# ErlerPhilipp/points2surf

Measured on AMD Instinct MI355X. Metric: SDF queries/sec/GPU (p2s_max, 256^3 grid), higher is better.
Workload: dtype f32

## Files before the change

### include/p2s_hip.h

```cpp
#ifndef P2S_HIP_H
#define P2S_HIP_H

#include <stddef.h>
#include <stdint.h>

#ifdef __cplusplus
extern "C" {
#endif

#define P2S_ABI_VERSION 5

#define P2S_OK            0
#define P2S_EINVAL       -1
#define P2S_EHIP         -2
#define P2S_ENOMEM       -3
#define P2S_ECAPACITY    -4
#define P2S_ENODEVICE    -5
#define P2S_EIO          -6

typedef struct p2s_model_s *p2s_model_t;
typedef struct p2s_cloud_s *p2s_cloud_t;
typedef struct p2s_rng_s   *p2s_rng_t;
typedef struct p2s_trimesh_s *p2s_trimesh_t;

// ... 125 lines not shown
    const p2s_rng_t *sub;
    const p2s_rng_t *first;
} p2s_worker_streams;
int p2s_stream_order(int64_t first_position, int64_t n, int n_streams, int batch, const float *q_in_dev, float *q_out_dev,
                     int64_t *src_out_dev, int64_t *counts_host, void *stream);
int p2s_infer_shape_workers(p2s_model_t m, p2s_cloud_t c, const p2s_worker_streams *ws, int grid_resolution, int epsilon,
                            int64_t q_begin, int64_t q_end, int chunk, float *sdf_out_dev, float *q_out_dev, int64_t *n_done,
                            void *stream);
int p2s_infer_queries_workers(p2s_model_t m, p2s_cloud_t c, const p2s_worker_streams *ws, int rotate, const float *q_dev,
                              int64_t n_queries, int chunk, float *sdf_out_dev, void *stream);
int p2s_subsample_workers(p2s_cloud_t c, const p2s_worker_streams *ws, const float *q_dev, int64_t n_queries, int n, int weighted,
                          int32_t *ids_out_dev, float *pts_out_dev, void *stream);
int p2s_model_capture_logits(p2s_model_t m, float *logits_out_dev, int64_t capacity_queries);
int p2s_debug_fault_chunk(p2s_model_t m, int chunk_index);
int p2s_debug_stn_pool(p2s_model_t m, int n_queries, float *out_dev, void *stream);

int p2s_sdf_volume(const float *query_dev, const float *sdf_dev, int64_t n, int grid_res, int sigma,
                   float certainty_threshold, int clamp, int device, float *vol_out_dev, int32_t *iterations,
                   void *stream);

int p2s_marching_cubes(const float *vol_dev, int grid_res, float *verts_out_dev, int64_t cap_verts,
                       int32_t *faces_out_dev, int64_t cap_faces, int64_t *n_verts, int64_t *n_faces,
                       int model_space, int fix_inversion, int *inverted, int device, void *stream);
int p2s_mc_cell(const float *values8, int32_t *row, int32_t *n_tri, int32_t *edges36);

int p2s_rng_random_sample(p2s_rng_t r, int64_t n, double *out_dev, void *stream);
int p2s_mesh_sample_surface(const float *verts_dev, const int32_t *faces_dev, int64_t n_faces, const double *u_dev,
                            int64_t n_samples, float *pts_out_dev, int32_t *face_out_dev, double *area_host,
                            int device, void *stream);
int p2s_points_remove_close(const float *pts_dev, int64_t m, double radius, int64_t limit, float *pts_out_dev,
// ... 61 lines not shown
                       int64_t *info_host, void *stream);

int p2s_write_txt_f32(const char *path, const float *values_host, int64_t n);
int p2s_write_query_vis_ply(const char *path, const float *query_host, const float *dist_host, int64_t n);
int p2s_write_coff_samples(const char *path, const float *query_host, const float *dist_host, int64_t n);

typedef struct {
    double  ms_chain_stn, ms_stn_head, ms_chain_main, ms_decoder, ms_knn, ms_subsample, ms_grid;
    int64_t queries;
    int64_t launches_chain;
    double  ms_chain_qstn;
    int64_t fallback_queries;
    int64_t conv3_confirmed;
    int64_t conv3_items_dense;
    int64_t conv3_items;
    double  reserved[3];
} p2s_counters;
int p2s_set_profiling(p2s_model_t m, int enabled);
int p2s_get_counters(p2s_model_t m, p2s_counters *out);

typedef struct p2s_trainer_s *p2s_trainer_t;

int p2s_trainer_create(const p2s_model_cfg *cfg, int use_feat_stn, const float *params_host, int64_t n_params,
                       const float *buffers_host, int64_t n_buffers, int64_t num_batches_tracked, int device,
                       p2s_trainer_t *out);
int p2s_trainer_destroy(p2s_trainer_t t);
int p2s_trainer_sizes(p2s_trainer_t t, int64_t *n_params, int64_t *n_buffers, int64_t *n_pools, int64_t *resident_bytes);
int p2s_trainer_forward_backward(p2s_trainer_t t, const float *patch_ps_dev, const float *sub_ms_dev, const float *query_dev,
                                 const float *dist_abs_dev, const float *sign01_dev, const float *radius_dev, int B,
                                 double *losses_host, void *stream);
int p2s_trainer_sgd_step(p2s_trainer_t t, double lr, double momentum, void *stream);
// ... 21 lines not shown
```

### points2surf_amd/_lib.py

```python
import ctypes
import os

from .weights import ModelCfg, WeightOffsets

HERE = os.path.dirname(os.path.abspath(__file__))
LIB_PATH = os.environ.get('P2S_LIB_PATH') or os.path.join(HERE, 'libp2s_hip.so')

P2S_OK = 0
P2S_ECAPACITY = -4

c_void_p = ctypes.c_void_p
c_int = ctypes.c_int
c_int64 = ctypes.c_int64


class Counters(ctypes.Structure):
    _fields_ = [('ms_chain_stn', ctypes.c_double), ('ms_stn_head', ctypes.c_double),
                ('ms_chain_main', ctypes.c_double), ('ms_decoder', ctypes.c_double),
                ('ms_knn', ctypes.c_double), ('ms_subsample', ctypes.c_double), ('ms_grid', ctypes.c_double),
                ('queries', ctypes.c_int64), ('launches_chain', ctypes.c_int64),
                ('ms_chain_qstn', ctypes.c_double), ('fallback_queries', ctypes.c_int64),
                ('conv3_confirmed', ctypes.c_int64), ('conv3_items_dense', ctypes.c_int64), ('conv3_items', ctypes.c_int64),
                ('reserved', ctypes.c_double * 3)]


PROTOTYPES = {
    'p2s_abi_version': (c_int, []),
    'p2s_last_error': (ctypes.c_char_p, []),
    'p2s_device_count': (c_int, []),
    'p2s_release_scratch': (c_int, [c_int]),
    'p2s_model_create': (c_int, [ctypes.POINTER(ModelCfg), c_void_p, ctypes.c_size_t,
                                 ctypes.POINTER(WeightOffsets), c_int, ctypes.POINTER(c_void_p)]),
    'p2s_model_destroy': (c_int, [c_void_p]),
    'p2s_encode_decode': (c_int, [c_void_p, c_void_p, c_void_p, c_void_p, c_void_p, c_int, c_void_p, c_void_p,
                                  c_void_p]),
    'p2s_encode_features': (c_int, [c_void_p, c_void_p, c_void_p, c_void_p, c_int, c_void_p, c_void_p, c_void_p]),
    'p2s_cloud_create': (c_int, [c_void_p, c_int, c_int, c_void_p, ctypes.POINTER(c_void_p)]),
    'p2s_cloud_destroy': (c_int, [c_void_p]),
# ... 16 lines not shown
    'p2s_patch_from_ids': (c_int, [c_void_p, c_void_p, c_void_p, c_void_p, c_int64, c_int, c_void_p, c_void_p, c_void_p]),
    'p2s_gather_points': (c_int, [c_void_p, c_void_p, c_int64, c_void_p, c_void_p]),
    'p2s_infer_shape': (c_int, [c_void_p, c_void_p, c_void_p, c_int, c_int, c_int64, c_int64, c_int, c_void_p,
                                c_void_p, ctypes.POINTER(c_int64), c_void_p]),
    'p2s_infer_shape_ball': (c_int, [c_void_p, c_void_p, c_void_p, c_void_p, c_int, c_int, c_int64, c_int64, c_int, c_void_p,
                                     c_void_p, ctypes.POINTER(c_int64), c_void_p]),
    'p2s_kd_order_host': (c_int, [c_void_p, c_int64, c_int, c_void_p, c_void_p, c_int64, ctypes.POINTER(ctypes.c_int32)]),
    'p2s_ball_count': (c_int, [c_void_p, c_void_p, c_int64, ctypes.c_double, c_void_p, c_void_p]),
    'p2s_ball_patch': (c_int, [c_void_p, c_void_p, c_void_p, c_int64, ctypes.c_double, c_int, c_int, c_void_p, c_void_p,
                               c_void_p, c_void_p, c_void_p]),
    'p2s_infer_queries': (c_int, [c_void_p, c_void_p, c_void_p, c_void_p, c_void_p, c_int64, c_int, c_void_p, c_void_p]),
    'p2s_random_rotations': (c_int, [c_void_p, c_int64, c_void_p, c_void_p]),
    'p2s_rotate_points': (c_int, [c_void_p, c_void_p, c_int, c_int64, c_void_p, c_void_p]),
    'p2s_debug_fault_chunk': (c_int, [c_void_p, c_int]),
    'p2s_debug_stn_pool': (c_int, [c_void_p, c_int, c_void_p, c_void_p]),
    'p2s_sdf_volume': (c_int, [c_void_p, c_void_p, c_int64, c_int, c_int, ctypes.c_float, c_int, c_int, c_void_p,
                               ctypes.POINTER(ctypes.c_int32), c_void_p]),
    'p2s_marching_cubes': (c_int, [c_void_p, c_int, c_void_p, c_int64, c_void_p, c_int64, ctypes.POINTER(c_int64),
                                   ctypes.POINTER(c_int64), c_int, c_int, ctypes.POINTER(c_int), c_int, c_void_p]),
    'p2s_mc_cell': (c_int, [c_void_p, ctypes.POINTER(ctypes.c_int32), ctypes.POINTER(ctypes.c_int32), c_void_p]),
    'p2s_rng_random_sample': (c_int, [c_void_p, c_int64, c_void_p, c_void_p]),
    'p2s_mesh_sample_surface': (c_int, [c_void_p, c_void_p, c_int64, c_void_p, c_int64, c_void_p, c_void_p,
                                        ctypes.POINTER(ctypes.c_double), c_int, c_void_p]),
    'p2s_points_remove_close': (c_int, [c_void_p, c_int64, ctypes.c_double, c_int64, c_void_p, ctypes.POINTER(c_int64), c_int,
                                        c_void_p]),
    'p2s_nn_distance_stats': (c_int, [c_void_p, c_void_p, c_int64, c_void_p, ctypes.POINTER(ctypes.c_double),
                                      ctypes.POINTER(ctypes.c_double), c_void_p]),
    'p2s_trimesh_create': (c_int, [c_void_p, c_int64, c_void_p, c_int64, c_int, c_void_p, ctypes.POINTER(c_void_p)]),
    'p2s_trimesh_destroy': (c_int, [c_void_p]),
    'p2s_trimesh_info': (c_int, [c_void_p, ctypes.POINTER(c_int64)]),
# ... 97 lines not shown
```

### points2surf_amd/build.py

```python
import glob
import os
import subprocess
import sys

HERE = os.path.dirname(os.path.abspath(__file__))
CSRC = os.path.join(HERE, 'csrc')
LIB = os.path.join(HERE, 'libp2s_hip.so')


def hipcc_path():
    for c in (os.environ.get('HIPCC'), '/opt/rocm/bin/hipcc', 'hipcc'):
        if c and (os.path.isfile(c) or c == 'hipcc'):
            return c
    return 'hipcc'


def sources():
    return sorted(glob.glob(os.path.join(CSRC, '*.hip')))


def needs_build():
    if not os.path.isfile(LIB):
        return True
    t = os.path.getmtime(LIB)
# ... 21 lines not shown
    tag = hashlib.sha1(' '.join(flags).encode()).hexdigest()[:10]
    todo, objs = [], []
    for src in sources():
        obj = os.path.join(objdir, '%s.%s.o' % (os.path.basename(src)[:-4], tag))
        objs.append(obj)
        if force or not os.path.isfile(obj) or os.path.getmtime(obj) < max(os.path.getmtime(src), hdr_time):
            todo.append((src, obj))

    def compile_one(job):
        src, obj = job
        cmd = [hipcc_path()] + flags + ['-c', src, '-o', obj]
        if verbose:
            print(' '.join(cmd), flush=True)
        subprocess.check_call(cmd)

    jobs = jobs or int(os.environ.get('P2S_BUILD_JOBS', min(8, os.cpu_count() or 1)))
    with concurrent.futures.ThreadPoolExecutor(max_workers=max(1, jobs)) as ex:
        list(ex.map(compile_one, todo))
    cmd = [hipcc_path(), '--offload-arch=gfx950', '-shared', '-fPIC', '-fno-gpu-rdc', '-o', LIB] + objs
    if verbose:
        print(' '.join(cmd), flush=True)
    subprocess.check_call(cmd)
    return LIB


if __name__ == '__main__':
    build(force='--force' in sys.argv)
    print(LIB)
```

### points2surf_amd/csrc/p2s_api.hip

```cpp
#include "p2s_common.h"
#include "p2s_internal.h"
#include <vector>
#include <cstring>
#include <algorithm>
#include <mutex>
#include <cstdlib>

static thread_local char g_err[512] = "";

void p2s_set_error(const char *fmt, ...) {
    va_list ap;
    va_start(ap, fmt);
    vsnprintf(g_err, sizeof(g_err), fmt, ap);
    va_end(ap);
}

namespace {
struct DevScratch {
    std::mutex mu;
    void *p = nullptr;
    size_t cap = 0;
};
DevScratch g_scratch[P2S_MAX_DEVICES];
}
// ... 58 lines not shown
    const p2s_model_cfg &cfg = m->cfg;
    hipError_t e = hipMalloc(&m->blob, n_floats * sizeof(float));
    if (e != hipSuccess) {
        p2s_set_error("hipMalloc(weights) failed: %s", hipGetErrorString(e));
        return P2S_ENOMEM;
    }
    e = hipMemcpy(m->blob, blob_host, n_floats * sizeof(float), hipMemcpyHostToDevice);
    if (e != hipSuccess) {
        p2s_set_error("hipMemcpy(weights) failed: %s", hipGetErrorString(e));
        return P2S_EHIP;
    }
    const Precision prec = p2s_precision(cfg);
    {
        const int rc = screen_init(m);
        if (rc) return rc;
    }
    if (!prec.pieces) return P2S_OK;
    struct Item { P2sLayer layer; int z; };
    std::vector<Item> items;
    for (int kind = LK_ENC; kind < LK_FP32; ++kind) {
        if (!p2s_kind_packed((P2sLayerKind)kind, cfg)) continue;
        const int slices = kind == LK_ENC || kind == LK_ENC_HEAD ? 2 : 1;
        for (int z = 0; z < slices; ++z)
            for (int l = 0; l < P2S_LAYERS; ++l) {
                if (p2s_layers[l].kind != kind) continue;
                m->h_off[l][z] = m->h_off[l][1] = m->h_total;
                items.push_back({(P2sLayer)l, z});
                m->h_total += (size_t)p2s_layers[l].K * p2s_layers[l].N;
            }
    }
// ... 123 lines not shown
    if (m->aux) (void)hipStreamDestroy(m->aux);
    if (m->ball) (void)hipStreamDestroy(m->ball);
    delete m;
    return P2S_OK;
}

int p2s_set_profiling(p2s_model_t m, int enabled) {
    if (!m) return P2S_EINVAL;
    m->profiling = enabled != 0;
    return P2S_OK;
}

int p2s_get_counters(p2s_model_t m, p2s_counters *out) {
    if (!m || !out) return P2S_EINVAL;
    *out = m->counters;
    if (m->scr_counters) {
        unsigned long long h[3] = {};
        P2S_HIP_CHECK(hipSetDevice(m->device));
        P2S_HIP_CHECK(hipMemcpy(h, m->scr_counters, sizeof(h), hipMemcpyDeviceToHost));
        out->conv3_confirmed = (int64_t)h[0];
        out->conv3_items_dense = (int64_t)h[1];
        out->conv3_items = (int64_t)h[2];
    }
    return P2S_OK;
}

}

int p2s_prof_mark(p2s_model_s *m, hipStream_t s) {
    if (!m->profiling) return -1;
// ... 132 lines not shown
```

### points2surf_amd/csrc/p2s_chain.hip

```cpp
#include "p2s_common.h"
#include <cstdlib>
#include <atomic>

namespace {

constexpr int MT = 64;
constexpr int SA = 68;
constexpr int SB = 132;

__device__ __forceinline__ f32x16 mfma32(float a, float b, f32x16 c) {
    return __builtin_amdgcn_mfma_f32_32x32x2f32(a, b, c, 0, 0, 0);
}

__device__ __forceinline__ f32x4 ldg4(const float *p) { return *reinterpret_cast<const f32x4 *>(p); }
__device__ __forceinline__ f32x4 lds4(const float *p) { return *reinterpret_cast<const f32x4 *>(p); }
__device__ __forceinline__ f32x4 bufld4(__amdgpu_buffer_rsrc_t rsrc, int voff, int soff) {
    typedef unsigned u32x4 __attribute__((ext_vector_type(4)));
    const u32x4 v = __builtin_amdgcn_raw_buffer_load_b128(rsrc, voff, soff, 0);
    f32x4 r;
    r[0] = __uint_as_float(v[0]); r[1] = __uint_as_float(v[1]); r[2] = __uint_as_float(v[2]); r[3] = __uint_as_float(v[3]);
    return r;
}

__device__ __forceinline__ void store_tile_bias_relu(const f32x16 &acc, float *dst, int stride, int row0,
                                                     int col0, const float *__restrict__ bias, int lane) {
    const int col = col0 + (lane & 31);
    const float b = bias[col];
    const int rbase = row0 + 4 * (lane >> 5);
#pragma unroll
    for (int reg = 0; reg < 16; ++reg) {
        const int row = rbase + (reg & 3) + 8 * (reg >> 2);
        dst[row * stride + col] = fmaxf(acc[reg] + b, 0.0f);
    }
}

__device__ __forceinline__ f32x16 zero16() {
    f32x16 z;
#pragma unroll
    for (int i = 0; i < 16; ++i) z[i] = 0.0f;
    return z;
}

struct B8 {
    f32x4 v[8];
};
__device__ __forceinline__ void load_b8(B8 &b, __amdgpu_buffer_rsrc_t rsrc, int lane16, int soff) {
#pragma unroll
    for (int kg = 0; kg < 8; ++kg) b.v[kg] = bufld4(rsrc, lane16, soff + kg * 1024);
// ... 103 lines not shown
    const auto r = __builtin_amdgcn_permlane32_swap(u, u, false, false);
    return __uint_as_float(r[0]) + __uint_as_float(r[1]);
}

typedef unsigned int u32x4 __attribute__((ext_vector_type(4)));
typedef _Float16 f16x8 __attribute__((ext_vector_type(8)));
typedef _Float16 f16x2 __attribute__((ext_vector_type(2)));
typedef float f32x2 __attribute__((ext_vector_type(2)));
constexpr int SCR_HB = 128 + 8;
constexpr int SCR_QCAP = 256;
constexpr float P2S_SCR_KAPPA = 0x1.1p-10f;
constexpr int SCR_OFF_E = MT * SA + MT * SB;
constexpr int SCR_OFF_Q = SCR_OFF_E + 1024;
constexpr int SCR_OFF_RED = SCR_OFF_Q + 4 * SCR_QCAP;
constexpr int SCR_LDS_FLOATS = SCR_OFF_RED + 8;
static_assert(MT * SCR_HB * 2 <= MT * SA * 4, "the fp16 copy fits the 64-channel tile it lies over");
static_assert(2 * SCR_LDS_FLOATS * 4 <= 160 * 1024, "two workgroups per CU");

__device__ __forceinline__ u32x4 scr_bufld(__amdgpu_buffer_rsrc_t rsrc, int voff, int soff) {
    return __builtin_amdgcn_raw_buffer_load_b128(rsrc, voff, soff, 0);
}
__device__ __forceinline__ u32x4 scr_lds_a(const unsigned short *buf, int row0, int kb, int lane) {
    return *reinterpret_cast<const u32x4 *>(buf + (row0 + (lane & 31)) * SCR_HB + 16 * kb + 8 * (lane >> 5));
}
__device__ __forceinline__ f32x16 scr_mfma(u32x4 a, u32x4 b, f32x16 c) {
    return __builtin_amdgcn_mfma_f32_32x32x16_f16(__builtin_bit_cast(f16x8, a), __builtin_bit_cast(f16x8, b), c, 0, 0, 0);
}
__device__ __forceinline__ unsigned scr_half2(float a, float b) {
    const f32x2 v = {a, b};
    return __builtin_bit_cast(unsigned, __builtin_convertvector(v, f16x2));
}
constexpr int SCR_CDEPTH = 4;
// ... 51 lines not shown
    const int wave = __builtin_amdgcn_readfirstlane(tid >> 6);

    int item = blockIdx.x;
    int bsel = 0;
    if (item >= args.br[0].n_items) {
        item -= args.br[0].n_items;
        bsel = 1;
    }
    const ChainBranch &br = args.br[bsel];
    const int P = br.P, P1 = br.P1;
    const float *__restrict__ w0a = br.w0a;
    const float *__restrict__ b0a = br.b0a;
    const float *__restrict__ w1 = br.w1 + (long long)item * br.w1_item_stride;
    const float *__restrict__ w3 = br.w3;
    const bool short_chain = br.short_chain != 0;

    float cx = 0.f, cy = 0.f, cz = 0.f;
    if (br.center) {
        cx = br.center[item * 3 + 0];
        cy = br.center[item * 3 + 1];
        cz = br.center[item * 3 + 2];
    }
    float R[9];
    const bool has_rot = br.rot != nullptr;
    if (has_rot) {
#pragma unroll
        for (int i = 0; i < 9; ++i) R[i] = br.rot[item * 9 + i];
    }

    const float pool0 = SUM ? 0.0f : -INFINITY;
// ... 31 lines not shown
    float *scr_red = smem + SCR_OFF_RED;
    unsigned *scr_q = reinterpret_cast<unsigned *>(smem + SCR_OFF_Q) + SCR_QCAP * wave;
    const float *__restrict__ scr_mu = args.w3mu[bsel];
    const __amdgpu_buffer_rsrc_t rs3h = __builtin_amdgcn_make_buffer_rsrc(const_cast<unsigned short *>(args.w3h[bsel]), 0,
                                                                           (int)(P2S_SCR_PIECE * 2), 0x00020000);
    float sr0 = -INFINITY, sr1 = -INFINITY, sr2 = -INFINITY, sr3 = -INFINITY, sr4 = -INFINITY, sr5 = -INFINITY, sr6 = -INFINITY,
          sr7 = -INFINITY;
    bool undec = false;
    float scr_Hsq = 0.0f;
    int nconf = 0;
    bool dense_pass = !SCREEN;
    if constexpr (SCREEN) {
#pragma unroll
        for (int i = 0; i < 4; ++i) scr_E[64 * i + lane] = __float_as_uint(-INFINITY);
    }
    for (;;) {
    load_point(0, nx0, nx1, nx2);
    for (int tile = 0; tile < ntiles; ++tile) {
      if constexpr (SCREEN) {
          asm volatile("" : "+v"(tid));
          lane = tid & 63;
          lane16 = lane * 16;
      }
      f32x4 bA0, bA1, aA0, aA1, bB0, bB1, aB0, aB1;
      if (ablate != 1) {
        float x0 = nx0, x1 = nx1, x2 = nx2;
        B8 wb;
        if (!short_chain) load_b8(wb, rs0b, lane16, (wave & 1) * 8192);
        else load_b8(wb, rs2, lane16, wave * 8192);
        if (has_rot) {
#pragma clang fp contract(off)
            const float y0 = __builtin_fmaf(R[0], x0, R[1] * x1) + R[2] * x2;
            const float y1 = __builtin_fmaf(R[5], x2, __builtin_fmaf(R[3], x0, R[4] * x1));
            const float y2 = __builtin_fmaf(R[8], x2, __builtin_fmaf(R[6], x0, R[7] * x1));
            x0 = y0; x1 = y1; x2 = y2;
        }
        bad = bad || !(fabsf(x0) <= 3.0e38f) || !(fabsf(x1) <= 3.0e38f) || !(fabsf(x2) <= 3.0e38f);
        {
            float *dst = bufA + lane * SA + 16 * wave;
#pragma unroll
            for (int c4 = 0; c4 < 4; ++c4) {
                f32x4 v;
#pragma unroll
                for (int c = 0; c < 4; ++c) {
                    const int o = 16 * wave + 4 * c4 + c;
                    float s = b0a[o];
                    s = fmaf(w0a[o], x0, s);
                    s = fmaf(w0a[64 + o], x1, s);
                    s = fmaf(w0a[128 + o], x2, s);
                    v[c] = fmaxf(s, 0.0f);
                }
                *reinterpret_cast<f32x4 *>(dst + 4 * c4) = v;
            }
        }
        __syncthreads();

        if (!short_chain) {
            {
                const int rt = wave >> 1, nt = wave & 1;
                f32x16 acc[1];
                layer_k64<1>(bufA, SA, 32 * rt, wb, lane, acc);
                load_b8(wb, rs1, lane16, nt * 8192);
                store_tile_bias_relu(acc[0], bufB, SB, 32 * rt, 32 * nt, br.b0b, lane);
            }
            __syncthreads();
            {
                const int rt = wave >> 1, nt = wave & 1;
                f32x16 acc[1];
                layer_k64<1>(bufB, SB, 32 * rt, wb, lane, acc);
                load_b8(wb, rs2, lane16, wave * 8192);
                store_tile_bias_relu(acc[0], bufA, SA, 32 * rt, 32 * nt, br.b1, lane);
            }
            __syncthreads();
        }
        {
            f32x16 acc[2];
            layer_k64<2>(bufA, SA, 0, wb, lane, acc);
            if (!SCREEN || dense_pass) {
                bA0 = bufld4(w3rsrc, lane16, w3soff);
                bA1 = bufld4(w3rsrc, lane16, w3soff + 16 * 1024);
            }
            store_tile_bias_relu(acc[0], bufB, SB, 0, 32 * wave, br.b2, lane);
            store_tile_bias_relu(acc[1], bufB, SB, 32, 32 * wave, br.b2, lane);
        }
        __syncthreads();
      } else {
        bA0 = bufld4(w3rsrc, lane16, w3soff);
        bA1 = bufld4(w3rsrc, lane16, w3soff + 16 * 1024);
      }
      if (ablate == 2) continue;
      if constexpr (SCREEN) {
        if (!dense_pass) {
#include "p2s_chain_screen.inl"
            continue;
        }
      }
        if (!SUM && tile == ntiles - 1 && P - tile * MT <= 48) {
#define P2S_TAIL 1
// ... 118 lines not shown
#ifdef P2S_DEV_ABLATE
    args.ablate = P2S_DEV_ABLATE + 0;
#endif
    const bool sum = args.br[0].pool_sum || (args.br[1].n_items > 0 && args.br[1].pool_sum);
    if (args.screen) {
        if (sum || args.br[0].short_chain || (args.br[1].n_items > 0 && args.br[1].short_chain) || !args.w3h[0] || !args.w3mu[0] ||
            (args.br[1].n_items > 0 && (!args.w3h[1] || !args.w3mu[1]))) {
            p2s_set_error("p2s_launch_chain: the screened conv3 takes full-chain max-pool passes with their screen operands");
            return P2S_EINVAL;
        }
        static std::atomic<bool> lds_set[P2S_MAX_DEVICES];
        int dev = 0;
        P2S_HIP_CHECK(hipGetDevice(&dev));
        if (dev < 0 || dev >= P2S_MAX_DEVICES || !lds_set[dev].load()) {
            const hipError_t attr = hipFuncSetAttribute((const void *)p2s_chain_kernel<false, true>,
                                                        hipFuncAttributeMaxDynamicSharedMemorySize, SCR_LDS_FLOATS * 4);
            if (attr != hipSuccess) {
                p2s_set_error("p2s_launch_chain: %d bytes of LDS for the screened conv3 refused: %s", SCR_LDS_FLOATS * 4, hipGetErrorString(attr));
                return P2S_EHIP;
            }
            if (dev >= 0 && dev < P2S_MAX_DEVICES) lds_set[dev].store(true);
        }
        hipLaunchKernelGGL((p2s_chain_kernel<false, true>), dim3(n), dim3(256), SCR_LDS_FLOATS * 4, stream, args);
    } else if (sum)
        hipLaunchKernelGGL(p2s_chain_kernel<true>, dim3(n), dim3(256), padlds, stream, args);
    else
        hipLaunchKernelGGL(p2s_chain_kernel<false>, dim3(n), dim3(256), padlds, stream, args);
    P2S_LAUNCH_CHECK("p2s_chain_kernel");
    return P2S_OK;
}

__global__ void p2s_screen_mu_kernel(const float *__restrict__ w3, float *__restrict__ mu) {
    const int c = blockIdx.x * blockDim.x + threadIdx.x;
    if (c >= 1024) return;
    double ss = 0.0;
    for (int g = 0; g < 16; ++g)
        for (int u = 0; u < 8; ++u) {
            const double w = w3[(((long long)(c >> 5) * 16 + g) * 64 + (u >> 2) * 32 + (c & 31)) * 4 + (u & 3)];
// ... 21 lines not shown
```

### points2surf_amd/csrc/p2s_common.h

```cpp
#pragma once
#include <hip/hip_runtime.h>
#include <cstdint>
#include <cstdio>
#include <cstdarg>
#include "../../include/p2s_hip.h"

typedef float f32x16 __attribute__((ext_vector_type(16)));
typedef float f32x4 __attribute__((ext_vector_type(4)));

__device__ __forceinline__ bool p2s_f16_out_of_range(float v) {
    const float a = fabsf(v);
    return a > 6.0e4f && a <= 3.4028235e38f;
}

void p2s_set_error(const char *fmt, ...);
constexpr int P2S_MAX_DEVICES = 16;
class P2sScratchLock {
public:
    explicit P2sScratchLock(int device);
    ~P2sScratchLock();
    P2sScratchLock(const P2sScratchLock &) = delete;
    P2sScratchLock &operator=(const P2sScratchLock &) = delete;
    void *get(size_t bytes);
private:
// ... 25 lines not shown
    const float *ptsB;
    const float *center;
    const float *rot;
    const float *w0a, *b0a;
    const float *w0b, *b0b;
    const float *w1, *b1;
    long long w1_item_stride;
    const float *w2, *b2;
    const float *w3, *b3;
    float *out;
    int P, P1;
    int n_items;
    int relu_out;
    int short_chain;
    int pool_sum;
};
struct ChainArgs {
    ChainBranch br[2];
    int ablate;
    int ns;
    long long piece_stride, w1_piece_stride;
    int f16;
    int *bad_items;
    int screen;
    const unsigned short *w3h[2];
    const float *w3mu[2];
    unsigned long long *scr_counters;
};
constexpr long long P2S_SCR_PIECE = 128 * 1024;
int p2s_launch_screen_prepare(const float *w32, unsigned short *dst, float *mu, hipStream_t stream, int *range_flag);
int p2s_launch_chain(const ChainArgs &args, hipStream_t stream);
// ... 37 lines not shown
```

### points2surf_amd/csrc/p2s_forward.hip

```cpp
#include "p2s_common.h"
#include "p2s_internal.h"
#include <cstring>
#include <algorithm>

namespace {

struct Ws {
    float *g_stn, *h1, *h2, *T, *w1p, *feat, *d1, *d2, *d3, *qg, *qg2, *qh1, *qh2, *rot;
    unsigned short *w1h;
    size_t floats;
};

Ws carve(float *base, const p2s_model_cfg &cfg, Precision prec, int C) {
    Ws w;
    size_t at = 0;
    auto take = [&](size_t n, bool present = true) {
        float *r = base && present ? base + at : nullptr; at += present ? n : 0; return r;
    };
    w.g_stn = take((size_t)2 * C * 1024);
    w.h1 = take((size_t)2 * C * 512);
    w.h2 = take((size_t)2 * C * 256);
    w.T = take((size_t)2 * C * 4096);
    w.w1p = take((size_t)2 * C * 4096);
    w.feat = take((size_t)2 * C * 1024);
    w.d1 = take((size_t)C * 1024);
    w.d2 = take((size_t)C * 256);
    w.d3 = take((size_t)C * 128);
    w.qg = take((size_t)C * 1024, cfg.use_point_stn);
    w.qg2 = take((size_t)C * 1024, cfg.use_point_stn);
    w.qh1 = take((size_t)C * 512, cfg.use_point_stn);
    w.qh2 = take((size_t)C * 256, cfg.use_point_stn);
    w.rot = take((size_t)C * 16, cfg.use_point_stn);
    w.w1h = reinterpret_cast<unsigned short *>(take((size_t)C * 4096 * prec.pieces, prec.pieces != 0));
    w.floats = at;
    return w;
}

struct Chunk {
    const p2s_model_s *m;
    Precision prec;
    const float *patch, *sub, *query, *rot;
    int C;
    Ws w;
};

const float *chain_operand(const unsigned short *h) { return reinterpret_cast<const float *>(h); }
const float *chain_operand(const Chunk &c, P2sLayer l, int e) { return c.prec.pieces ? chain_operand(c.m->w16(l, e)) : c.m->w32(l, e); }

enum Pass { PASS_QSTN, PASS_STN, PASS_MAIN };

void fill_branch(ChainBranch &b, const Chunk &c, Pass pass, int e) {
    const p2s_model_s *m = c.m;
    const float *W = m->blob;
    const p2s_encoder_offsets &eo = m->offs.enc[e];
    const size_t C = c.C;
    if (e == 1) { b.ptsA = nullptr; b.ptsB = c.sub; b.center = c.query; b.P = m->cfg.sub_sample_size; b.P1 = 0; }
    else        { b.ptsA = c.patch; b.ptsB = nullptr; b.center = nullptr; b.P = b.P1 = m->cfg.points_per_patch; }
    b.n_items = c.C;
    b.rot = c.rot;
    b.relu_out = pass != PASS_MAIN;
    b.short_chain = pass == PASS_QSTN;
    b.pool_sum = pass == PASS_MAIN && m->cfg.sym_sum;
    const P2sLayer l2 = pass == PASS_QSTN ? L_QC2 : pass == PASS_STN ? L_S2 : L_M2;
    const P2sLayer l3 = pass == PASS_QSTN ? L_QC3 : pass == PASS_STN ? L_S3 : L_M3;
    const int z = pass == PASS_QSTN ? 0 : e;
    b.w2 = chain_operand(c, l2, z); b.b2 = m->bias(l2, z);
    b.w3 = chain_operand(c, l3, z); b.b3 = m->bias(l3, z);
    if (pass == PASS_QSTN) {
        b.w0a = W + m->offs.qstn.c1; b.b0a = W + m->offs.qstn.cb1;
        b.w0b = b.b0b = nullptr; b.w1 = W; b.b1 = nullptr; b.w1_item_stride = 0;
        b.out = e == 1 ? c.w.qg : c.w.qg2;
        return;
    }
    b.w0a = W + eo.w0a; b.b0a = W + eo.b0a;
    b.w0b = chain_operand(c, L_W0B, e); b.b0b = m->bias(L_W0B, e);
    if (pass == PASS_STN) {
        b.w1 = chain_operand(c, L_S1, e); b.b1 = m->bias(L_S1, e); b.w1_item_stride = 0;
// ... 34 lines not shown
    const bool h16 = c.prec.f16 && d.kind != LK_FP32;
    for (int z = 0; z < 2; ++z) {
        g.W[z] = c.m->w32(layer, z);
        g.bias[z] = c.m->bias(layer, z);
        g.Wh[z] = h16 ? c.m->w16(layer, z) : nullptr;
    }
    g.wh_piece = h16 ? (long long)c.m->h_total : 0;
    g.bad_rows = h16 ? c.m->fb.flags : nullptr;
    g.A = A; g.lda = d.K; g.a_z = g.Z == 2 ? (long long)c.C * d.K : 0;
    g.C = out; g.ldc = ldc; g.c_z = c_z; g.N = d.N; g.K = d.K;
    return p2s_launch_gemm(g, s);
}

}

int p2s_model_reserve(p2s_model_s *m, int chunk) {
    if (chunk <= m->ws_chunk) return P2S_OK;
    if (m->ws) {
        P2S_HIP_CHECK(hipDeviceSynchronize());
        (void)hipFree(m->ws);
        m->ws = nullptr;
        m->ws_chunk = 0;
    }
    const size_t n = carve(nullptr, m->cfg, p2s_precision(m->cfg), 1).floats * (size_t)chunk;
    hipError_t e = hipMalloc(&m->ws, n * sizeof(float));
    if (e != hipSuccess) {
        p2s_set_error("hipMalloc(workspace %zu MB) failed: %s", n * 4 >> 20, hipGetErrorString(e));
        return P2S_ENOMEM;
    }
    m->ws_chunk = chunk;
    return P2S_OK;
}

__global__ __launch_bounds__(256) void p2s_fb_collect_kernel(int *__restrict__ flags, int *__restrict__ count, int cap,
                                                             const float *__restrict__ patch, const float *__restrict__ sub,
                                                             const float *__restrict__ query, const float *__restrict__ radius,
                                                             int k3, int n3, long long index0, float *__restrict__ fpatch,
                                                             float *__restrict__ fsub, float *__restrict__ fquery,
                                                             float *__restrict__ fradius, long long *__restrict__ findex) {
    __shared__ int s_slot;
// ... 22 lines not shown
                                      const float *__restrict__ logits, int n, int od, float *__restrict__ sdf_out,
                                      float *__restrict__ logits_out) {
    const int i = blockIdx.x * blockDim.x + threadIdx.x;
    if (i >= n) return;
    const long long d = index[i];
    if (sdf_out) sdf_out[d] = sdf[i];
    if (logits_out)
        for (int j = 0; j < od; ++j) logits_out[d * od + j] = logits[(size_t)i * od + j];
}

int p2s_run_chunk(p2s_model_s *m, Precision prec, const float *patch, const float *sub, const float *query, const float *radius,
                  int C, float *logits_out, float *sdf_out, float *feat_local_out, float *feat_global_out,
                  hipStream_t s, long long index0) {
    const p2s_weight_offsets &o = m->offs;
    const float *W = m->blob;
    Chunk c = {m, prec, patch, sub, query, nullptr, C, carve(m->ws, m->cfg, prec, C)};
    const Ws &w = c.w;
    int rc;
    const int ev0 = p2s_prof_mark(m, s);
    int evq1 = -1, evq2 = -1;

    if (m->cfg.use_point_stn) {
        const bool qstn_shared = m->cfg.shared_transformer != 0 || m->cfg.single_transformer != 0;
        ChainArgs a = chain_args(c);
        fill_branch(a.br[0], c, PASS_QSTN, 1);
        fill_branch(a.br[1], c, PASS_QSTN, qstn_shared ? 0 : 1);
        if (!qstn_shared) a.br[1].n_items = 0;
        if ((rc = launch_chain(a, c, s))) return rc;
        evq1 = p2s_prof_mark(m, s);
        m->counters.launches_chain += 1;
        GemmArgs g;
        memset(&g, 0, sizeof(g));
// ... 77 lines not shown
    p2s_prof_span(m, ST_DECODER, ev3, ev4);
    if (prec.f16 && m->fb.flags) {
        hipLaunchKernelGGL(p2s_fb_collect_kernel, dim3(C), dim3(256), 0, s, m->fb.flags, m->fb.count, m->fb.cap, patch, sub, query,
                           radius, m->cfg.points_per_patch * 3, m->cfg.sub_sample_size * 3, index0, m->fb.patch, m->fb.sub, m->fb.query, m->fb.radius, m->fb.index);
        P2S_LAUNCH_CHECK("p2s_fb_collect_kernel");
    }
    return P2S_OK;
}

extern "C" int p2s_debug_stn_pool(p2s_model_t m, int n_queries, float *out_dev, void *stream) {
    if (!m || !out_dev || n_queries < 1 || n_queries > m->ws_chunk || n_queries > m->max_chunk) {
        p2s_set_error("p2s_debug_stn_pool: no workspace of a call of %d queries (one internal batch)", n_queries);
        return P2S_EINVAL;
    }
    P2S_HIP_CHECK(hipSetDevice(m->device));
    const Ws w = carve(m->ws, m->cfg, p2s_precision(m->cfg), n_queries);
    P2S_HIP_CHECK(hipMemcpyAsync(out_dev, w.g_stn, (size_t)2 * n_queries * 1024 * sizeof(float), hipMemcpyDeviceToDevice, (hipStream_t)stream));
    return P2S_OK;
}

int p2s_fallback_finish(p2s_model_s *m, float *logits_out, float *sdf_out, hipStream_t s) {
    p2s_model_s::Fallback &fb = m->fb;
    if (!fb.count) return P2S_OK;
    int h = 0;
    P2S_HIP_CHECK(hipMemcpyAsync(&h, fb.count, 4, hipMemcpyDeviceToHost, s));
    P2S_HIP_CHECK(hipStreamSynchronize(s));
    if (!h) return P2S_OK;
    if (h > fb.cap || (!logits_out && !sdf_out)) {
        p2s_set_error("fp16 pair encoder (encoder_bf16 = 4): %d queries of this call have activations beyond the half range (> 6e4)%s "
                      "-- use encoder_bf16 = 3 or 0 for this model", h,
                      h > fb.cap ? ", more than the fp32 fallback takes per call (16384)" : " and the call has no output the fp32 fallback could repair");
// ... 18 lines not shown
```

### points2surf_amd/csrc/p2s_internal.h

```cpp
#pragma once
#include "p2s_common.h"
#include <vector>
#include <cstddef>

struct PipeBuffers {
    float *patch[2] = {};
    float *radius[2] = {};
    int32_t *sub_ids[2] = {};
    float *sub[2] = {};
    float *qrot[2] = {};
    double *rot[2] = {};
    hipEvent_t ready[2] = {};
    hipEvent_t freed[2] = {};
    hipEvent_t done[2] = {};
    hipEvent_t ball_ready[2] = {};
    hipEvent_t grid = nullptr;
    int32_t *knn_ids[2] = {};
    int32_t *perm[2] = {};
    int cap_chunk = 0, cap_k = 0, cap_n = 0, cap_small = 0;
};

struct Precision {
    int pieces;
    bool f16;
// ... 48 lines not shown
    unsigned long long *scr_counters = nullptr;
    const unsigned short *screen_w(P2sLayer layer, int z) const { return scr_w3h + ((layer == L_M3 ? 2 : 0) + z) * P2S_SCR_PIECE; }
    const float *screen_mu(P2sLayer layer, int z) const { return scr_mu + ((layer == L_M3 ? 2 : 0) + z) * 1024; }
    struct Fallback {
        int *flags = nullptr;
        int *count = nullptr;
        float *patch = nullptr, *sub = nullptr, *query = nullptr, *radius = nullptr;
        long long *index = nullptr;
        float *sdf = nullptr, *logits = nullptr;
        int cap = 0;
    } fb;
    float *logits_capture = nullptr;
    int64_t logits_capacity = 0;
    float *ws = nullptr;
    int ws_chunk = 0;
    int max_chunk = 8192;
    bool profiling = false;
    std::vector<hipEvent_t> evpool;
    int ev_used = 0;
    struct Span { int stage, a, b; };
    std::vector<Span> spans;
    p2s_counters counters = {};
    hipStream_t aux = nullptr;
    hipStream_t ball = nullptr;
    bool overlap = true;
    PipeBuffers pipe;
    int fault_chunk = -1;
    struct Workers {
        float *q = nullptr, *sdf = nullptr, *logits = nullptr;
        int64_t *src = nullptr;
// ... 20 lines not shown
    const hipStream_t s;
    const bool pipeline;
    float *logits = nullptr;
    int64_t logits_room = 0;
    int rc = P2S_OK;
    ModelCall(p2s_model_s *m, hipStream_t s, bool pipeline);
    int fail(int code);
    int finish(float *logits_out, float *sdf_out, int64_t nq);
};

enum P2SStage { ST_CHAIN_STN = 0, ST_HEAD, ST_CHAIN_MAIN, ST_DECODER, ST_KNN, ST_SUB, ST_GRID, ST_CHAIN_QSTN };
int p2s_prof_mark(p2s_model_s *m, hipStream_t s);
void p2s_prof_span(p2s_model_s *m, int stage, int a, int b);

int p2s_model_reserve(p2s_model_s *m, int chunk);
int p2s_run_chunk(p2s_model_s *m, Precision prec, const float *patch, const float *sub, const float *query, const float *radius,
                  int C, float *logits_out, float *sdf_out, float *feat_local_out, float *feat_global_out,
                  hipStream_t s, long long index0 = 0);
int p2s_fallback_finish(p2s_model_s *m, float *logits_out, float *sdf_out, hipStream_t s);

struct CloudDev {
    const float *pts;
    const float4 *spts;
    const int *cell_start;
    const int *sat;
    float lo[3];
    float inv_cell;
    int G;
    int n;
};
// ... 110 lines not shown
```

Measured before the change: 446,000.

## Cache STN-pass stem activations and reuse them in the main encoder pass

The STN pass of the screened chain kernel writes its conv0 (stem) output tiles to a new global workspace buffer. The main pass then streams those tiles back into LDS with LDS-DMA, prefetching the next tile during conv2, and skips recomputing conv0. This removes the duplicated first-layer work at the cost of extra workspace memory, global traffic and a larger LDS footprint, with a recompute fallback when allocation fails or an environment flag is set.

Measured after the change: 435,200. 2.4% lower.

```diff
diff --git a/include/p2s_hip.h b/include/p2s_hip.h
--- a/include/p2s_hip.h
+++ b/include/p2s_hip.h
@@ -163,6 +163,7 @@
 int p2s_model_capture_logits(p2s_model_t m, float *logits_out_dev, int64_t capacity_queries);
 int p2s_debug_fault_chunk(p2s_model_t m, int chunk_index);
 int p2s_debug_stn_pool(p2s_model_t m, int n_queries, float *out_dev, void *stream);
+int p2s_debug_workspace_layout(const p2s_model_cfg *cfg, int chunk, int with_stem, int64_t *out);
 
 int p2s_sdf_volume(const float *query_dev, const float *sdf_dev, int64_t n, int grid_res, int sigma,
                    float certainty_threshold, int clamp, int device, float *vol_out_dev, int32_t *iterations,
@@ -254,7 +255,8 @@
     int64_t conv3_confirmed;
     int64_t conv3_items_dense;
     int64_t conv3_items;
-    double  reserved[3];
+    int64_t stem_bytes;
+    double  reserved[2];
 } p2s_counters;
 int p2s_set_profiling(p2s_model_t m, int enabled);
 int p2s_get_counters(p2s_model_t m, p2s_counters *out);
diff --git a/points2surf_amd/_lib.py b/points2surf_amd/_lib.py
--- a/points2surf_amd/_lib.py
+++ b/points2surf_amd/_lib.py
@@ -21,7 +21,7 @@
                 ('queries', ctypes.c_int64), ('launches_chain', ctypes.c_int64),
                 ('ms_chain_qstn', ctypes.c_double), ('fallback_queries', ctypes.c_int64),
                 ('conv3_confirmed', ctypes.c_int64), ('conv3_items_dense', ctypes.c_int64), ('conv3_items', ctypes.c_int64),
-                ('reserved', ctypes.c_double * 3)]
+                ('stem_bytes', ctypes.c_int64), ('reserved', ctypes.c_double * 2)]
 
 
 PROTOTYPES = {
@@ -68,6 +68,7 @@
     'p2s_rotate_points': (c_int, [c_void_p, c_void_p, c_int, c_int64, c_void_p, c_void_p]),
     'p2s_debug_fault_chunk': (c_int, [c_void_p, c_int]),
     'p2s_debug_stn_pool': (c_int, [c_void_p, c_int, c_void_p, c_void_p]),
+    'p2s_debug_workspace_layout': (c_int, [ctypes.POINTER(ModelCfg), c_int, c_int, ctypes.POINTER(c_int64)]),
     'p2s_sdf_volume': (c_int, [c_void_p, c_void_p, c_int64, c_int, c_int, ctypes.c_float, c_int, c_int, c_void_p,
                                ctypes.POINTER(ctypes.c_int32), c_void_p]),
     'p2s_marching_cubes': (c_int, [c_void_p, c_int, c_void_p, c_int64, c_void_p, c_int64, ctypes.POINTER(c_int64),
diff --git a/points2surf_amd/build.py b/points2surf_amd/build.py
--- a/points2surf_amd/build.py
+++ b/points2surf_amd/build.py
@@ -59,7 +59,7 @@
             print(' '.join(cmd), flush=True)
         subprocess.check_call(cmd)
 
-    jobs = jobs or int(os.environ.get('P2S_BUILD_JOBS', min(8, os.cpu_count() or 1)))
+    jobs = jobs or int(os.environ.get('MAX_JOBS') or min(8, os.cpu_count() or 1))
     with concurrent.futures.ThreadPoolExecutor(max_workers=max(1, jobs)) as ex:
         list(ex.map(compile_one, todo))
     cmd = [hipcc_path(), '--offload-arch=gfx950', '-shared', '-fPIC', '-fno-gpu-rdc', '-o', LIB] + objs
diff --git a/points2surf_amd/csrc/p2s_api.hip b/points2surf_amd/csrc/p2s_api.hip
--- a/points2surf_amd/csrc/p2s_api.hip
+++ b/points2surf_amd/csrc/p2s_api.hip
@@ -96,6 +96,8 @@
     {
         const int rc = screen_init(m);
         if (rc) return rc;
+        const char *recompute = getenv("P2S_STEM_RECOMPUTE");
+        m->stem_recompute = recompute && atoi(recompute) != 0;
     }
     if (!prec.pieces) return P2S_OK;
     struct Item { P2sLayer layer; int z; };
@@ -249,6 +251,7 @@
 int p2s_get_counters(p2s_model_t m, p2s_counters *out) {
     if (!m || !out) return P2S_EINVAL;
     *out = m->counters;
+    out->stem_bytes = (int64_t)p2s_stem_bytes(m);
     if (m->scr_counters) {
         unsigned long long h[3] = {};
         P2S_HIP_CHECK(hipSetDevice(m->device));
diff --git a/points2surf_amd/csrc/p2s_chain.hip b/points2surf_amd/csrc/p2s_chain.hip
--- a/points2surf_amd/csrc/p2s_chain.hip
+++ b/points2surf_amd/csrc/p2s_chain.hip
@@ -23,15 +23,19 @@
 }
 
 __device__ __forceinline__ void store_tile_bias_relu(const f32x16 &acc, float *dst, int stride, int row0,
-                                                     int col0, const float *__restrict__ bias, int lane) {
+                                                     int col0, float b, int lane) {
     const int col = col0 + (lane & 31);
-    const float b = bias[col];
     const int rbase = row0 + 4 * (lane >> 5);
 #pragma unroll
     for (int reg = 0; reg < 16; ++reg) {
         const int row = rbase + (reg & 3) + 8 * (reg >> 2);
         dst[row * stride + col] = fmaxf(acc[reg] + b, 0.0f);
     }
+}
+
+__device__ __forceinline__ void store_tile_bias_relu(const f32x16 &acc, float *dst, int stride, int row0,
+                                                     int col0, const float *__restrict__ bias, int lane) {
+    store_tile_bias_relu(acc, dst, stride, row0, col0, bias[col0 + (lane & 31)], lane);
 }
 
 __device__ __forceinline__ f32x16 zero16() {
@@ -165,8 +169,12 @@
 constexpr int SCR_OFF_Q = SCR_OFF_E + 1024;
 constexpr int SCR_OFF_RED = SCR_OFF_Q + 4 * SCR_QCAP;
 constexpr int SCR_LDS_FLOATS = SCR_OFF_RED + 8;
+constexpr int SCR_OFF_STEM = SCR_LDS_FLOATS;
+constexpr int SCR_LDS_FLOATS_STEM = SCR_OFF_STEM + P2S_STEM_TILE_FLOATS;
+static_assert(P2S_STEM_TILE_FLOATS == MT * SA && P2S_STEM_TILE_FLOATS % 256 == 0, "the stem tile is conv1's LDS image, whole wave instructions");
+static_assert(SCR_OFF_STEM % 4 == 0, "16-byte LDS-DMA destinations");
 static_assert(MT * SCR_HB * 2 <= MT * SA * 4, "the fp16 copy fits the 64-channel tile it lies over");
-static_assert(2 * SCR_LDS_FLOATS * 4 <= 160 * 1024, "two workgroups per CU");
+static_assert(2 * SCR_LDS_FLOATS_STEM * 4 <= 160 * 1024, "two workgroups per CU");
 
 __device__ __forceinline__ u32x4 scr_bufld(__amdgpu_buffer_rsrc_t rsrc, int voff, int soff) {
     return __builtin_amdgcn_raw_buffer_load_b128(rsrc, voff, soff, 0);
@@ -248,6 +256,8 @@
     const float *__restrict__ w1 = br.w1 + (long long)item * br.w1_item_stride;
     const float *__restrict__ w3 = br.w3;
     const bool short_chain = br.short_chain != 0;
+    const bool stem_wr = SCREEN && br.stem_role == P2S_STEM_WRITE;
+    const bool stem_rd = SCREEN && br.stem_role == P2S_STEM_READ;
 
     float cx = 0.f, cy = 0.f, cz = 0.f;
     if (br.center) {
@@ -309,8 +319,26 @@
 #pragma unroll
         for (int i = 0; i < 4; ++i) scr_E[64 * i + lane] = __float_as_uint(-INFINITY);
     }
+    auto stem_fetch = [&](int t) {
+        if constexpr (SCREEN) {
+            const float *g = br.stem + ((long long)item * ntiles + t) * P2S_STEM_TILE_FLOATS + lane * 4;
+            float *l = smem + SCR_OFF_STEM;
+#pragma unroll
+            for (int j = 0; j < 5; ++j) {
+                const int k = wave + 4 * j;
+                if (k < P2S_STEM_TILE_FLOATS / 256)
+                    __builtin_amdgcn_global_load_lds((const __attribute__((address_space(1))) void *)(g + k * 256),
+                                                     (__attribute__((address_space(3))) void *)(l + k * 256), 16, 0, 0);
+            }
+        }
+    };
     for (;;) {
     load_point(0, nx0, nx1, nx2);
+    if (stem_rd) {
+        stem_fetch(0);
+        asm volatile("s_waitcnt vmcnt(0)" ::: "memory");
+        __syncthreads();
+    }
     for (int tile = 0; tile < ntiles; ++tile) {
       if constexpr (SCREEN) {
           asm volatile("" : "+v"(tid));
@@ -320,8 +348,12 @@
       f32x4 bA0, bA1, aA0, aA1, bB0, bB1, aB0, aB1;
       if (ablate != 1) {
         float x0 = nx0, x1 = nx1, x2 = nx2;
-        B8 wb;
-        if (!short_chain) load_b8(wb, rs0b, lane16, (wave & 1) * 8192);
+        B8 wb, wb2;
+        float b2v;
+        const bool abl_stem = ablate == 6 && br.w1_item_stride != 0 && !stem_rd;
+        const bool no_stem = stem_rd;
+        if (no_stem || abl_stem) load_b8(wb, rs1, lane16, (wave & 1) * 8192);
+        else if (!short_chain) load_b8(wb, rs0b, lane16, (wave & 1) * 8192);
         else load_b8(wb, rs2, lane16, wave * 8192);
         if (has_rot) {
 #pragma clang fp contract(off)
@@ -331,8 +363,8 @@
             x0 = y0; x1 = y1; x2 = y2;
         }
         bad = bad || !(fabsf(x0) <= 3.0e38f) || !(fabsf(x1) <= 3.0e38f) || !(fabsf(x2) <= 3.0e38f);
-        {
-            float *dst = bufA + lane * SA + 16 * wave;
+        if (!no_stem) {
+            float *dst = abl_stem ? bufB + lane * SB + 16 * wave : bufA + lane * SA + 16 * wave;
 #pragma unroll
             for (int c4 = 0; c4 < 4; ++c4) {
                 f32x4 v;
@@ -348,35 +380,55 @@
                 *reinterpret_cast<f32x4 *>(dst + 4 * c4) = v;
             }
         }
-        __syncthreads();
+        if (!no_stem) __syncthreads();
 
         if (!short_chain) {
-            {
+            if (!no_stem && !abl_stem) {
                 const int rt = wave >> 1, nt = wave & 1;
                 f32x16 acc[1];
                 layer_k64<1>(bufA, SA, 32 * rt, wb, lane, acc);
                 load_b8(wb, rs1, lane16, nt * 8192);
                 store_tile_bias_relu(acc[0], bufB, SB, 32 * rt, 32 * nt, br.b0b, lane);
-            }
-            __syncthreads();
+                __syncthreads();
+                if (stem_wr) {
+                    float *g = br.stem + ((long long)item * ntiles + tile) * P2S_STEM_TILE_FLOATS;
+#pragma unroll
+                    for (int j = 0; j < 4; ++j) {
+                        const int i = tid + 256 * j, row = i >> 4, c4 = i & 15;
+                        *reinterpret_cast<f32x4 *>(g + row * SA + 4 * c4) = lds4(bufB + row * SB + 4 * c4);
+                    }
+                }
+            }
             {
                 const int rt = wave >> 1, nt = wave & 1;
                 f32x16 acc[1];
-                layer_k64<1>(bufB, SB, 32 * rt, wb, lane, acc);
-                load_b8(wb, rs2, lane16, wave * 8192);
+                if (stem_rd) b2v = br.b2[32 * wave + (lane & 31)];
+                layer_k64<1>(stem_rd ? smem + SCR_OFF_STEM : bufB, stem_rd ? SA : SB, 32 * rt, wb, lane, acc);
+                load_b8(wb2, rs2, lane16, wave * 8192);
                 store_tile_bias_relu(acc[0], bufA, SA, 32 * rt, 32 * nt, br.b1, lane);
             }
             __syncthreads();
-        }
-        {
+        } else {
+            wb2 = wb;
+        }
+        auto conv2 = [&]() {
             f32x16 acc[2];
-            layer_k64<2>(bufA, SA, 0, wb, lane, acc);
+            layer_k64<2>(bufA, SA, 0, wb2, lane, acc);
             if (!SCREEN || dense_pass) {
                 bA0 = bufld4(w3rsrc, lane16, w3soff);
                 bA1 = bufld4(w3rsrc, lane16, w3soff + 16 * 1024);
             }
-            store_tile_bias_relu(acc[0], bufB, SB, 0, 32 * wave, br.b2, lane);
-            store_tile_bias_relu(acc[1], bufB, SB, 32, 32 * wave, br.b2, lane);
+            store_tile_bias_relu(acc[0], bufB, SB, 0, 32 * wave, b2v, lane);
+            store_tile_bias_relu(acc[1], bufB, SB, 32, 32 * wave, b2v, lane);
+        };
+        if (stem_rd) {
+            __builtin_amdgcn_s_waitcnt(0x0F70);
+            if (tile + 1 < ntiles) stem_fetch(tile + 1);
+            conv2();
+            __builtin_amdgcn_s_waitcnt(0x0F70);
+        } else {
+            b2v = br.b2[32 * wave + (lane & 31)];
+            conv2();
         }
         __syncthreads();
       } else {
@@ -525,14 +577,20 @@
         P2S_HIP_CHECK(hipGetDevice(&dev));
         if (dev < 0 || dev >= P2S_MAX_DEVICES || !lds_set[dev].load()) {
             const hipError_t attr = hipFuncSetAttribute((const void *)p2s_chain_kernel<false, true>,
-                                                        hipFuncAttributeMaxDynamicSharedMemorySize, SCR_LDS_FLOATS * 4);
+                                                        hipFuncAttributeMaxDynamicSharedMemorySize, SCR_LDS_FLOATS_STEM * 4);
             if (attr != hipSuccess) {
-                p2s_set_error("p2s_launch_chain: %d bytes of LDS for the screened conv3 refused: %s", SCR_LDS_FLOATS * 4, hipGetErrorString(attr));
+                p2s_set_error("p2s_launch_chain: %d bytes of LDS for the screened conv3 refused: %s", SCR_LDS_FLOATS_STEM * 4, hipGetErrorString(attr));
                 return P2S_EHIP;
             }
             if (dev >= 0 && dev < P2S_MAX_DEVICES) lds_set[dev].store(true);
         }
-        hipLaunchKernelGGL((p2s_chain_kernel<false, true>), dim3(n), dim3(256), SCR_LDS_FLOATS * 4, stream, args);
+        const bool rd = args.br[0].stem_role == P2S_STEM_READ || (args.br[1].n_items > 0 && args.br[1].stem_role == P2S_STEM_READ);
+        for (int b = 0; b < 2; ++b)
+            if (args.br[b].n_items > 0 && args.br[b].stem_role != P2S_STEM_NONE && !args.br[b].stem) {
+                p2s_set_error("p2s_launch_chain: a stem role without a stem buffer");
+                return P2S_EINVAL;
+            }
+        hipLaunchKernelGGL((p2s_chain_kernel<false, true>), dim3(n), dim3(256), (rd ? SCR_LDS_FLOATS_STEM : SCR_LDS_FLOATS) * 4, stream, args);
     } else if (sum)
         hipLaunchKernelGGL(p2s_chain_kernel<true>, dim3(n), dim3(256), padlds, stream, args);
     else
diff --git a/points2surf_amd/csrc/p2s_common.h b/points2surf_amd/csrc/p2s_common.h
--- a/points2surf_amd/csrc/p2s_common.h
+++ b/points2surf_amd/csrc/p2s_common.h
@@ -63,7 +63,11 @@
     int relu_out;
     int short_chain;
     int pool_sum;
+    float *stem;
+    int stem_role;
 };
+enum { P2S_STEM_NONE = 0, P2S_STEM_WRITE = 1, P2S_STEM_READ = 2 };
+constexpr int P2S_STEM_TILE_FLOATS = 64 * 68;
 struct ChainArgs {
     ChainBranch br[2];
     int ablate;
diff --git a/points2surf_amd/csrc/p2s_forward.hip b/points2surf_amd/csrc/p2s_forward.hip
--- a/points2surf_amd/csrc/p2s_forward.hip
+++ b/points2surf_amd/csrc/p2s_forward.hip
@@ -1,17 +1,23 @@
 #include "p2s_common.h"
 #include "p2s_internal.h"
 #include <cstring>
+#include <cstdio>
+#include <atomic>
 #include <algorithm>
 
 namespace {
 
 struct Ws {
     float *g_stn, *h1, *h2, *T, *w1p, *feat, *d1, *d2, *d3, *qg, *qg2, *qh1, *qh2, *rot;
+    float *stem;
     unsigned short *w1h;
     size_t floats;
+    size_t stem_at, stem_floats, w1h_at, w1h_floats;
 };
 
-Ws carve(float *base, const p2s_model_cfg &cfg, Precision prec, int C) {
+int stem_tiles(const p2s_model_cfg &cfg, int e) { return ((e == 1 ? cfg.sub_sample_size : cfg.points_per_patch) + 63) / 64; }
+
+Ws carve(float *base, const p2s_model_cfg &cfg, Precision prec, int C, bool stem) {
     Ws w;
     size_t at = 0;
     auto take = [&](size_t n, bool present = true) {
@@ -31,7 +37,12 @@
     w.qh1 = take((size_t)C * 512, cfg.use_point_stn);
     w.qh2 = take((size_t)C * 256, cfg.use_point_stn);
     w.rot = take((size_t)C * 16, cfg.use_point_stn);
+    w.stem_at = at;
+    w.stem = take((size_t)C * (stem_tiles(cfg, 0) + stem_tiles(cfg, 1)) * P2S_STEM_TILE_FLOATS, stem);
+    w.stem_floats = at - w.stem_at;
+    w.w1h_at = at;
     w.w1h = reinterpret_cast<unsigned short *>(take((size_t)C * 4096 * prec.pieces, prec.pieces != 0));
+    w.w1h_floats = at - w.w1h_at;
     w.floats = at;
     return w;
 }
@@ -42,6 +53,7 @@
     const float *patch, *sub, *query, *rot;
     int C;
     Ws w;
+    bool stem;
 };
 
 const float *chain_operand(const unsigned short *h) { return reinterpret_cast<const float *>(h); }
@@ -61,6 +73,12 @@
     b.relu_out = pass != PASS_MAIN;
     b.short_chain = pass == PASS_QSTN;
     b.pool_sum = pass == PASS_MAIN && m->cfg.sym_sum;
+    b.stem = nullptr;
+    b.stem_role = P2S_STEM_NONE;
+    if (c.stem && pass != PASS_QSTN) {
+        b.stem = c.w.stem + (e == 1 ? C * stem_tiles(m->cfg, 0) * P2S_STEM_TILE_FLOATS : 0);
+        b.stem_role = pass == PASS_STN ? P2S_STEM_WRITE : P2S_STEM_READ;
+    }
     const P2sLayer l2 = pass == PASS_QSTN ? L_QC2 : pass == PASS_STN ? L_S2 : L_M2;
     const P2sLayer l3 = pass == PASS_QSTN ? L_QC3 : pass == PASS_STN ? L_S3 : L_M3;
     const int z = pass == PASS_QSTN ? 0 : e;
@@ -125,6 +143,27 @@
 
 }
 
+bool p2s_stem_wanted(const p2s_model_s *m) {
+    return m->cfg.encoder_bf16 == 0 && m->scr_w3h && !m->cfg.sym_sum && !m->stem_recompute && !m->stem_failed;
+}
+size_t p2s_stem_bytes(const p2s_model_s *m) {
+    return m->stem_on ? carve(nullptr, m->cfg, p2s_precision(m->cfg), m->ws_chunk, true).stem_floats * sizeof(float) : 0;
+}
+
+extern "C" int p2s_debug_workspace_layout(const p2s_model_cfg *cfg, int chunk, int with_stem, int64_t *out) {
+    if (!cfg || !out || chunk < 1 || cfg->points_per_patch < 1 || cfg->sub_sample_size < 1 || cfg->encoder_bf16 < 0 || cfg->encoder_bf16 > 4) {
+        p2s_set_error("p2s_debug_workspace_layout: bad argument");
+        return P2S_EINVAL;
+    }
+    const Ws w = carve(nullptr, *cfg, p2s_precision(*cfg), chunk, with_stem != 0);
+    out[0] = (int64_t)(w.floats * 4);
+    out[1] = (int64_t)(w.stem_at * 4);
+    out[2] = (int64_t)(w.stem_floats * 4);
+    out[3] = (int64_t)(w.w1h_at * 4);
+    out[4] = (int64_t)(w.w1h_floats * 4);
+    return P2S_OK;
+}
+
 int p2s_model_reserve(p2s_model_s *m, int chunk) {
     if (chunk <= m->ws_chunk) return P2S_OK;
     if (m->ws) {
@@ -133,8 +172,23 @@
         m->ws = nullptr;
         m->ws_chunk = 0;
     }
-    const size_t n = carve(nullptr, m->cfg, p2s_precision(m->cfg), 1).floats * (size_t)chunk;
+    m->stem_on = false;
+    bool stem = p2s_stem_wanted(m);
+    size_t n = carve(nullptr, m->cfg, p2s_precision(m->cfg), 1, stem).floats * (size_t)chunk;
     hipError_t e = hipMalloc(&m->ws, n * sizeof(float));
+    if (e != hipSuccess && stem) {
+        (void)hipGetLastError();
+        m->ws = nullptr;
+        static std::atomic<bool> said;
+        if (!said.exchange(true))
+            fprintf(stderr, "points2surf_amd: no room for the stem buffer (workspace of %zu MB: %s); the main pass recomputes the stem\n",
+                    n * 4 >> 20, hipGetErrorString(e));
+        m->stem_failed = true;
+        stem = false;
+        n = carve(nullptr, m->cfg, p2s_precision(m->cfg), 1, false).floats * (size_t)chunk;
+        e = hipMalloc(&m->ws, n * sizeof(float));
+    }
+    m->stem_on = stem && e == hipSuccess;
     if (e != hipSuccess) {
         p2s_set_error("hipMalloc(workspace %zu MB) failed: %s", n * 4 >> 20, hipGetErrorString(e));
         return P2S_ENOMEM;
@@ -187,8 +241,9 @@
                   hipStream_t s, long long index0) {
     const p2s_weight_offsets &o = m->offs;
     const float *W = m->blob;
-    Chunk c = {m, prec, patch, sub, query, nullptr, C, carve(m->ws, m->cfg, prec, C)};
+    Chunk c = {m, prec, patch, sub, query, nullptr, C, carve(m->ws, m->cfg, prec, C, m->stem_on), false};
     const Ws &w = c.w;
+    c.stem = w.stem && prec.pieces == 0 && m->scr_w3h && !m->cfg.sym_sum;
     int rc;
     const int ev0 = p2s_prof_mark(m, s);
     int evq1 = -1, evq2 = -1;
@@ -296,7 +351,7 @@
         return P2S_EINVAL;
     }
     P2S_HIP_CHECK(hipSetDevice(m->device));
-    const Ws w = carve(m->ws, m->cfg, p2s_precision(m->cfg), n_queries);
+    const Ws w = carve(m->ws, m->cfg, p2s_precision(m->cfg), n_queries, m->stem_on);
     P2S_HIP_CHECK(hipMemcpyAsync(out_dev, w.g_stn, (size_t)2 * n_queries * 1024 * sizeof(float), hipMemcpyDeviceToDevice, (hipStream_t)stream));
     return P2S_OK;
 }
diff --git a/points2surf_amd/csrc/p2s_internal.h b/points2surf_amd/csrc/p2s_internal.h
--- a/points2surf_amd/csrc/p2s_internal.h
+++ b/points2surf_amd/csrc/p2s_internal.h
@@ -86,6 +86,9 @@
     int64_t logits_capacity = 0;
     float *ws = nullptr;
     int ws_chunk = 0;
+    bool stem_recompute = false;
+    bool stem_failed = false;
+    bool stem_on = false;
     int max_chunk = 8192;
     bool profiling = false;
     std::vector<hipEvent_t> evpool;
@@ -136,6 +139,8 @@
 void p2s_prof_span(p2s_model_s *m, int stage, int a, int b);
 
 int p2s_model_reserve(p2s_model_s *m, int chunk);
+bool p2s_stem_wanted(const p2s_model_s *m);
+size_t p2s_stem_bytes(const p2s_model_s *m);
 int p2s_run_chunk(p2s_model_s *m, Precision prec, const float *patch, const float *sub, const float *query, const float *radius,
                   int C, float *logits_out, float *sdf_out, float *feat_local_out, float *feat_global_out,
                   hipStream_t s, long long index0 = 0);
```
